# dalek-cryptography/curve25519-dalek

Measured on NVIDIA H100. Metric: Pippenger MSM points/sec, higher is better.
Workload: dtype exact integers: f64 limbs (radix 2^51, FP64 pipe) in the bucket kernel, u32 limbs (radix 2^25.5) elsewhere

## Files before the change

### curve25519_dalek_b200/csrc/fe64.cuh

```cuda
#pragma once
#include <stdint.h>

#include "fe.cuh"

struct fe64 { double v[5]; };

#define FE64_E52 0x4330000000000000LL
#define FE64_TWO52 4503599627370496.0
#define FE64_TWO51 2251799813685248.0

#if defined(__CUDA_ARCH__)
#define FE64_DEV 1
#else
#define FE64_DEV 0
#include <assert.h>
#include <math.h>
#include <string.h>
#endif

FE_HD void fe64_0(fe64 &h) { for (int i = 0; i < 5; i++) h.v[i] = 0.0; }
FE_HD void fe64_1(fe64 &h) { h.v[0] = 1.0; for (int i = 1; i < 5; i++) h.v[i] = 0.0; }

FE_HD void fe64_add(fe64 &h, const fe64 &f, const fe64 &g)
{
#pragma unroll
    for (int i = 0; i < 5; i++) h.v[i] = f.v[i] + g.v[i];
}
FE_HD void fe64_sub(fe64 &h, const fe64 &f, const fe64 &g)
{
#pragma unroll
    for (int i = 0; i < 5; i++) h.v[i] = f.v[i] - g.v[i];
}

FE_HD void fe64_cmov(fe64 &h, const fe64 &g, uint32_t c)
{
#if FE64_DEV
#pragma unroll
    for (int i = 0; i < 5; i++) {
        long long a = __double_as_longlong(h.v[i]), b = __double_as_longlong(g.v[i]);
        long long m = 0LL - (long long)c;
        h.v[i] = __longlong_as_double(a ^ (m & (a ^ b)));
    }
#else
    if (c) h = g;
#endif
}

#if !FE64_DEV
static inline void fe64_assert_scale(const fe64 &f, double s)
{
    for (int i = 0; i < 5; i++) {
        assert(f.v[i] == floor(f.v[i]));
        assert(fabs(f.v[i]) <= s * 1125899906842624.0 + 32768.0 * s);
    }
}
#define FE64_ASSERT_SCALE(f, s) fe64_assert_scale((f), (s))
#else
#define FE64_ASSERT_SCALE(f, s) ((void)0)
#endif

FE_HD void fe64_finish(fe64 &h, long long V[9])
{
    long long R[5];
#pragma unroll
    for (int k = 0; k < 4; k++) R[k] = V[k] + 19 * V[k + 5];
    R[4] = V[4];
    const long long HALF = 1LL << 50;
    long long c;
    c = (R[0] + HALF) >> 51; R[0] -= c * (1LL << 51); R[1] += c;
    c = (R[1] + HALF) >> 51; R[1] -= c * (1LL << 51); R[2] += c;
    c = (R[2] + HALF) >> 51; R[2] -= c * (1LL << 51); R[3] += c;
    c = (R[3] + HALF) >> 51; R[3] -= c * (1LL << 51); R[4] += c;
    c = (R[4] + HALF) >> 51; R[4] -= c * (1LL << 51); R[0] += 19 * c;
    c = (R[0] + HALF) >> 51; R[0] -= c * (1LL << 51); R[1] += c;
#pragma unroll
    for (int k = 0; k < 5; k++) {
#if FE64_DEV
        h.v[k] = __longlong_as_double((R[k] + (1LL << 51)) | FE64_E52) - (FE64_TWO52 + FE64_TWO51);
#else
        h.v[k] = (double)R[k];
#endif
    }
}

FE_HD void fe64_mul(fe64 &h, const fe64 &a, const fe64 &b)
{
    long long V[9];
#if FE64_DEV
    const double M1 = 6755399441055744.0;
    const double K = 6755399441055744.0 * 4503599627370496.0 + 4503599627370496.0;
    double bs[5];
#pragma unroll
    for (int j = 0; j < 5; j++) bs[j] = b.v[j] * (1.0 / 4503599627370496.0);
    long long H[10], L[9];
#pragma unroll
    for (int k = 0; k < 10; k++) H[k] = 0;
#pragma unroll
    for (int k = 0; k < 9; k++) L[k] = 0;
#pragma unroll
    for (int i = 0; i < 5; i++)
#pragma unroll
        for (int j = 0; j < 5; j++) {
            double t = __fma_rz(a.v[i], bs[j], M1);
            double u = __fma_rn(t, -4503599627370496.0, K);
            double lo = __fma_rn(a.v[i], b.v[j], u);
            H[i + j + 1] += __double_as_longlong(t);
            L[i + j] += __double_as_longlong(lo);
        }
    const long long EH = FE64_E52 + (1LL << 51);
#pragma unroll
    for (int k = 0; k < 9; k++) {
        const int nl = k < 5 ? k + 1 : 9 - k;
        const int nh = k == 0 ? 0 : (k <= 5 ? k : 10 - k);
        V[k] = (L[k] - nl * FE64_E52) + 2 * (H[k] - nh * EH);
    }
    V[4] += 38 * (H[9] - EH);
#else
    for (int k = 0; k < 9; k++) V[k] = 0;
    long long V9 = 0;
    for (int i = 0; i < 5; i++)
        for (int j = 0; j < 5; j++) {
            __int128 p = (__int128)(long long)a.v[i] * (__int128)(long long)b.v[j];
            __int128 lim = (__int128)1 << 103;
            assert(p < lim && p > -lim);
            long long f = (long long)(p >> 52);
            long long lo = (long long)(p - ((__int128)f << 52));
            V[i + j] += lo;
            if (i + j + 1 < 9) V[i + j + 1] += 2 * f; else V9 += 2 * f;
        }
    V[4] += 19 * V9;
#endif
    fe64_finish(h, V);
}

FE_HD void fe64_sq(fe64 &h, const fe64 &a)
{
    long long V[9];
#if FE64_DEV
    const double M1 = 6755399441055744.0;
    const double K = 6755399441055744.0 * 4503599627370496.0 + 4503599627370496.0;
    double as[5], a2[5];
#pragma unroll
    for (int j = 0; j < 5; j++) { as[j] = a.v[j] * (1.0 / 4503599627370496.0); a2[j] = a.v[j] + a.v[j]; }
    long long H[10], L[9];
#pragma unroll
    for (int k = 0; k < 10; k++) H[k] = 0;
#pragma unroll
    for (int k = 0; k < 9; k++) L[k] = 0;
#pragma unroll
    for (int i = 0; i < 5; i++)
#pragma unroll
        for (int j = i; j < 5; j++) {
            const double x = i < j ? a2[i] : a.v[i];
            double t = __fma_rz(x, as[j], M1);
            double u = __fma_rn(t, -4503599627370496.0, K);
            double lo = __fma_rn(x, a.v[j], u);
            H[i + j + 1] += __double_as_longlong(t);
            L[i + j] += __double_as_longlong(lo);
        }
    const long long EH = FE64_E52 + (1LL << 51);
#pragma unroll
    for (int k = 0; k < 9; k++) {
        const int nl = k < 5 ? k / 2 + 1 : (8 - k) / 2 + 1;
        const int km = k - 1;
        const int nh = k == 0 ? 0 : (km < 5 ? km / 2 + 1 : (8 - km) / 2 + 1);
        V[k] = (L[k] - nl * FE64_E52) + 2 * (H[k] - nh * EH);
    }
    V[4] += 38 * (H[9] - EH);
#else
    for (int k = 0; k < 9; k++) V[k] = 0;
    long long V9 = 0;
    for (int i = 0; i < 5; i++)
        for (int j = i; j < 5; j++) {
            __int128 p = (__int128)(long long)a.v[i] * (__int128)(long long)a.v[j] * (i < j ? 2 : 1);
            __int128 lim = (__int128)1 << 103;
            assert(p < lim && p > -lim);
            long long f = (long long)(p >> 52);
            long long lo = (long long)(p - ((__int128)f << 52));
            V[i + j] += lo;
            if (i + j + 1 < 9) V[i + j + 1] += 2 * f; else V9 += 2 * f;
        }
    V[4] += 19 * V9;
#endif
    fe64_finish(h, V);
}

FE_HD void fe64_sqn(fe64 &h, const fe64 &f, int n)
{
    fe64_sq(h, f);
#if FE64_DEV
#pragma unroll 1
#endif
    for (int i = 1; i < n; i++) fe64_sq(h, h);
}

FE_HD void fe64_carry(fe64 &h, const fe64 &f)
{
#if FE64_DEV
    const double C = 6755399441055744.0;
    double q[5], r[5];
#pragma unroll
    for (int k = 0; k < 5; k++) {
        q[k] = __fma_rn(f.v[k], 1.0 / 2251799813685248.0, C) - C;
        r[k] = __fma_rn(q[k], -2251799813685248.0, f.v[k]);
    }
    h.v[0] = __fma_rn(q[4], 19.0, r[0]);
#pragma unroll
    for (int k = 1; k < 5; k++) h.v[k] = r[k] + q[k - 1];
#else
    double q[5], r[5];
    for (int k = 0; k < 5; k++) { q[k] = nearbyint(f.v[k] / 2251799813685248.0); r[k] = f.v[k] - q[k] * 2251799813685248.0; }
    h.v[0] = r[0] + 19.0 * q[4];
    for (int k = 1; k < 5; k++) h.v[k] = r[k] + q[k - 1];
#endif
}

FE_HD void fe64_frombytes_words(fe64 &h, const uint32_t w[8])
{
    uint64_t l[5];
    l[0] = (uint64_t)w[0] | ((uint64_t)(w[1] & 0x7ffffu) << 32);
    l[1] = (uint64_t)(w[1] >> 19) | ((uint64_t)w[2] << 13) | ((uint64_t)(w[3] & 0x3fu) << 45);
    l[2] = (uint64_t)(w[3] >> 6) | ((uint64_t)(w[4] & 0x1ffffffu) << 26);
    l[3] = (uint64_t)(w[4] >> 25) | ((uint64_t)w[5] << 7) | ((uint64_t)(w[6] & 0xfffu) << 39);
    l[4] = (uint64_t)(w[6] >> 12) | ((uint64_t)(w[7] & 0x7fffffffu) << 20);
#pragma unroll
    for (int k = 0; k < 5; k++) {
#if FE64_DEV
        h.v[k] = __longlong_as_double((long long)l[k] | FE64_E52) - FE64_TWO52;
#else
        h.v[k] = (double)l[k];
#endif
    }
}

FE_HD void fe64_to_fe(fe &o, const fe64 &f)
{
    uint64_t l[5];
#pragma unroll
    for (int k = 0; k < 5; k++) {
        long long r = (long long)f.v[k];
        l[k] = (uint64_t)(r + (k == 0 ? (1LL << 54) - 152 : (1LL << 54) - 8));
    }
    uint64_t c[10];
#pragma unroll
    for (int i = 0; i < 5; i++) { c[2 * i] = l[i] & FE_M26; c[2 * i + 1] = l[i] >> 26; }
    fe_carry64(o, c);
}

FE_HD void fe64_from_fe(fe64 &h, const fe &f)
{
    uint32_t w[8];
    fe_tobytes_words(w, f);
    fe64 t; fe64_frombytes_words(t, w);
    fe64_carry(h, t);
}

FE_HD void fe64_pow22501(fe64 &t19, fe64 &t3, const fe64 &z)
{
    fe64 t0, t1, t2, t5, t6, t7, t9, t13, t15;
    fe64_sq(t0, z);
    fe64_sqn(t1, t0, 2);
    fe64_mul(t2, z, t1);
    fe64_mul(t3, t0, t2);
    fe64_sq(t1, t3);
    fe64_mul(t5, t2, t1);
    fe64_sqn(t6, t5, 5);    fe64_mul(t7, t6, t5);
    fe64_sqn(t6, t7, 10);   fe64_mul(t9, t6, t7);
    fe64_sqn(t6, t9, 20);   fe64_mul(t6, t6, t9);
    fe64_sqn(t6, t6, 10);   fe64_mul(t13, t6, t7);
    fe64_sqn(t6, t13, 50);  fe64_mul(t15, t6, t13);
    fe64_sqn(t6, t15, 100); fe64_mul(t6, t6, t15);
    fe64_sqn(t6, t6, 50);   fe64_mul(t19, t6, t13);
}

FE_HD void fe_pow_p58_f64(fe &h, const fe &f)
{
    fe64 z, t19, t3;
    fe64_from_fe(z, f);
    fe64_pow22501(t19, t3, z);
    fe64_sqn(t19, t19, 2);
    fe64_mul(t19, z, t19);
    fe64_to_fe(h, t19);
}

FE_HD void fe_invert_f64(fe &h, const fe &f)
{
    fe64 z, t19, t3;
    fe64_from_fe(z, f);
    fe64_pow22501(t19, t3, z);
    fe64_sqn(t19, t19, 5);
    fe64_mul(t19, t19, t3);
    fe64_to_fe(h, t19);
}
```

### curve25519_dalek_b200/csrc/ge64.cuh

```cuda
#pragma once
#include "fe64.cuh"
#include "ge.cuh"

struct ge64_p3 { fe64 X, Y, Z, T; };
struct ge64_niels { fe64 ypx, ymx, xy2d; };
struct ge64_pniels { fe64 YpX, YmX, Z, T2d; };

FE_HD void ge64_identity(ge64_p3 &p) { fe64_0(p.X); fe64_1(p.Y); fe64_1(p.Z); fe64_0(p.T); }

FE_HD void ge64_niels_unpack(ge64_niels &n, const ge_niels_packed &o)
{
    fe64_frombytes_words(n.ypx, o.w); fe64_frombytes_words(n.ymx, o.w + 8); fe64_frombytes_words(n.xy2d, o.w + 16);
}
FE_HD void ge64_pniels_unpack(ge64_pniels &n, const ge_pniels_packed &o)
{
    fe64_frombytes_words(n.YpX, o.w); fe64_frombytes_words(n.YmX, o.w + 8);
    fe64_frombytes_words(n.Z, o.w + 16); fe64_frombytes_words(n.T2d, o.w + 24);
}

FE_HD void ge64_add_tail(ge64_p3 &r, const fe64 &a, const fe64 &b, const fe64 &c, const fe64 &D, uint32_t neg)
{
    fe64 E, H, DpC, DmC, F, G;
    fe64_sub(E, b, a);
    fe64_add(H, b, a);
    fe64_add(DpC, D, c);
    fe64_sub(DmC, D, c);
    fe64_carry(DmC, DmC);
    F = DmC; fe64_cmov(F, DpC, neg);
    G = DpC; fe64_cmov(G, DmC, neg);
    fe64_mul(r.X, F, E);
    fe64_mul(r.Y, G, H);
    fe64_mul(r.Z, DmC, DpC);
    fe64_mul(r.T, E, H);
}

FE_HD void ge64_madd(ge64_p3 &r, const ge64_p3 &p, const ge64_niels &q, uint32_t neg)
{
    FE64_ASSERT_SCALE(p.X, 1); FE64_ASSERT_SCALE(p.Y, 1); FE64_ASSERT_SCALE(p.Z, 1); FE64_ASSERT_SCALE(p.T, 1);
    fe64 A, B, a, b, c, D;
    fe64 qp = q.ypx, qm = q.ymx;
    { fe64 t = qp; fe64_cmov(qp, qm, neg); fe64_cmov(qm, t, neg); }
    fe64_sub(A, p.Y, p.X);
    fe64_add(B, p.Y, p.X);
    fe64_mul(a, A, qm);
    fe64_mul(b, B, qp);
    fe64_mul(c, p.T, q.xy2d);
    fe64_add(D, p.Z, p.Z);
    ge64_add_tail(r, a, b, c, D, neg);
}

FE_HD void ge64_padd(ge64_p3 &r, const ge64_p3 &p, const ge64_pniels &q, uint32_t neg)
{
    FE64_ASSERT_SCALE(p.X, 1); FE64_ASSERT_SCALE(p.Y, 1); FE64_ASSERT_SCALE(p.Z, 1); FE64_ASSERT_SCALE(p.T, 1);
    fe64 A, B, a, b, c, ZZ, D;
    fe64 qp = q.YpX, qm = q.YmX;
    { fe64 t = qp; fe64_cmov(qp, qm, neg); fe64_cmov(qm, t, neg); }
    fe64_sub(A, p.Y, p.X);
    fe64_add(B, p.Y, p.X);
    fe64_mul(a, A, qm);
    fe64_mul(b, B, qp);
    fe64_mul(c, p.T, q.T2d);
    fe64_mul(ZZ, p.Z, q.Z);
    fe64_add(D, ZZ, ZZ);
    ge64_add_tail(r, a, b, c, D, neg);
}

template <bool T_OUT = true>
FE_HD void ge64_dbl(ge64_p3 &r, const ge64_p3 &p)
{
    FE64_ASSERT_SCALE(p.X, 1); FE64_ASSERT_SCALE(p.Y, 1); FE64_ASSERT_SCALE(p.Z, 1);
    fe64 XX, YY, ZZ, XpY, XpY2, Yp, Ym, E, F;
    fe64_sq(XX, p.X);
    fe64_sq(YY, p.Y);
    fe64_sq(ZZ, p.Z);
    fe64_add(XpY, p.X, p.Y); fe64_carry(XpY, XpY);
    fe64_sq(XpY2, XpY);
    fe64_add(Yp, YY, XX);
    fe64_sub(Ym, YY, XX);
    fe64_sub(E, XpY2, Yp);
    fe64_add(F, ZZ, ZZ); fe64_sub(F, F, Ym);
    fe64_carry(F, F);
    fe64_mul(r.X, E, F);
    fe64_mul(r.Y, Yp, Ym);
    fe64_mul(r.Z, Ym, F);
    if (T_OUT) fe64_mul(r.T, E, Yp);
}

FE_HD void ge64_add_p3(ge64_p3 &r, const ge64_p3 &p, const ge64_p3 &q, const fe64 &d2)
{
    ge64_pniels pn;
    fe64_add(pn.YpX, q.Y, q.X);
    fe64_sub(pn.YmX, q.Y, q.X);
    pn.Z = q.Z;
    fe64_mul(pn.T2d, q.T, d2);
    ge64_padd(r, p, pn, 0u);
}

FE_HD void ge64_from_p3(ge64_p3 &o, const ge_p3 &p)
{
    fe64_from_fe(o.X, p.X); fe64_from_fe(o.Y, p.Y); fe64_from_fe(o.Z, p.Z); fe64_from_fe(o.T, p.T);
}

FE_HD void ge64_to_p3(ge_p3 &o, const ge64_p3 &p)
{
    fe64_to_fe(o.X, p.X); fe64_to_fe(o.Y, p.Y); fe64_to_fe(o.Z, p.Z); fe64_to_fe(o.T, p.T);
}
```

### curve25519_dalek_b200/csrc/msm.cu

```cuda
#include <algorithm>
#include <cstdio>
#include <utility>
#include <vector>

#include "../../include/dalek_b200.h"
#include "engine.h"
#include "ge64.cuh"
#include "warp4.cuh"
#include "warp4_f64.cuh"

static inline unsigned cdiv(size_t a, unsigned b) { return (unsigned)((a + b - 1) / b); }

int ws_reserve(dalek_b200_ctx *ctx, DevBuf &b, size_t bytes)
{
    if (bytes <= b.cap) return 0;
    if (b.p) { cudaFree(b.p); b.p = nullptr; b.cap = 0; }
    size_t want = bytes + bytes / 8 + 256;
    cudaError_t e = cudaMalloc(&b.p, want);
    if (e != cudaSuccess) {
        ctx->last_error = std::string("cudaMalloc: ") + cudaGetErrorString(e);
        (void)cudaGetLastError();
        return DALEK_E_NOMEM;
    }
    b.cap = want;
// ... 496 lines not shown
{
    extern __shared__ uint32_t sm[];
    __shared__ uint32_t s_bin, s_slice;
    uint2 *recs = reinterpret_cast<uint2 *>(sm);
    uint32_t *out = sm + 2 * SORT_FINE_CAP, *h = out + SORT_FINE_CAP, *scr = h + (1u << F);
    const uint32_t nf = 1u << F, nbins = nwin * nc;
    uint32_t bin, slice = 0;
    if (blockIdx.x < nbins) {
        bin = nbins - 1 - blockIdx.x;
    } else {
        if (threadIdx.x == 0) {
            uint32_t t = blockIdx.x - nbins, w = 0;
            while (w < nwin && t >= xtot[w]) t -= xtot[w++];
            s_bin = nbins;
            if (w < nwin) {
                const uint32_t *x = xpre + (size_t)w * nc;
                uint32_t lo = 0, hi = nc - 1;
                while (lo < hi) { const uint32_t mid = (lo + hi + 1) / 2; if (x[mid] <= t) lo = mid; else hi = mid - 1; }
                s_bin = w * nc + lo;
                s_slice = t - x[lo] + 1;
            }
        }
        __syncthreads();
        bin = s_bin; slice = s_slice;
        if (bin >= nbins) return;
    }
    const uint32_t wb = bin / nc, cb = bin % nc;
    const uint32_t cnt = ccount[bin], base = ccursor[bin] - cnt;
    const size_t seg = flat ? (size_t)0 : (size_t)wb * n;
    const size_t b0 = (size_t)wb * nbuckets + ((size_t)cb << F);
    const uint2 *src = records + seg + base;
    uint32_t *dst = sorted + seg + base;
    constexpr uint32_t U = 4;
    if (cnt <= SORT_FINE_CAP) {
        for (uint32_t f = threadIdx.x; f < nf; f += SORT_THREADS) h[f] = 0;
        __syncthreads();
        for (uint32_t k0 = 0; k0 < cnt; k0 += U * SORT_THREADS) {
            uint2 r[U];
#pragma unroll
            for (uint32_t u = 0; u < U; u++) {
                const uint32_t k = k0 + u * SORT_THREADS + threadIdx.x;
                r[u] = k < cnt ? src[k] : make_uint2(0, 0);
            }
#pragma unroll
            for (uint32_t u = 0; u < U; u++) {
                const uint32_t k = k0 + u * SORT_THREADS + threadIdx.x;
                if (k < cnt) { recs[k] = r[u]; atomicAdd(&h[r[u].y], 1u); }
            }
        }
        __syncthreads();
        for (uint32_t f = threadIdx.x; f < nf; f += SORT_THREADS) counts[b0 + f] = h[f];
        block_excl_scan(h, nf, scr);
        for (uint32_t f = threadIdx.x; f < nf; f += SORT_THREADS) offsets[b0 + f] = base + h[f];
        __syncthreads();
        for (uint32_t k = threadIdx.x; k < cnt; k += SORT_THREADS) { const uint2 r = recs[k]; out[atomicAdd(&h[r.y], 1u)] = r.x; }
        __syncthreads();
        for (uint32_t k = threadIdx.x; k < cnt; k += SORT_THREADS) dst[k] = out[k];
        return;
    }
    for (uint32_t f = threadIdx.x; f < nf; f += SORT_THREADS) { h[f] = counts[b0 + f]; out[f] = 0; }
    block_excl_scan(h, nf, scr);
    if (slice == 0)
        for (uint32_t f = threadIdx.x; f < nf; f += SORT_THREADS) offsets[b0 + f] = base + h[f];
    const uint32_t lo = slice * SORT_FINE_CAP, m = min(SORT_FINE_CAP, cnt - lo);
    for (uint32_t k0 = 0; k0 < m; k0 += U * SORT_THREADS) {
        uint2 r[U];
#pragma unroll
        for (uint32_t u = 0; u < U; u++) {
            const uint32_t k = k0 + u * SORT_THREADS + threadIdx.x;
            r[u] = k < m ? src[lo + k] : make_uint2(0, 0);
        }
#pragma unroll
        for (uint32_t u = 0; u < U; u++) {
            const uint32_t k = k0 + u * SORT_THREADS + threadIdx.x;
            if (k < m) recs[k] = r[u];
            warp_claim(out, r[u].y, k < m);
        }
    }
    __syncthreads();
    for (uint32_t f = threadIdx.x; f < nf; f += SORT_THREADS)
        if (out[f]) out[f] = h[f] + atomicAdd(&fill[b0 + f], out[f]);
    __syncthreads();
    for (uint32_t k0 = 0; k0 < m; k0 += SORT_THREADS) {
        const uint32_t k = k0 + threadIdx.x;
        const uint2 r = k < m ? recs[k] : make_uint2(0, 0);
        const uint32_t pos = warp_claim(out, r.y, k < m);
        if (k < m) dst[pos] = r.x;
    }
}

#define SCAN_PART 4096u
__global__ void __launch_bounds__(1024) k_scan_partial(const uint32_t *__restrict__ in, uint32_t nbuckets, uint32_t parts,
                                                       uint32_t *__restrict__ part_sums)
{
    __shared__ uint32_t sh[32];
    uint32_t w = blockIdx.x / parts, part = blockIdx.x % parts;
    const uint32_t *src = in + (size_t)w * nbuckets;
    uint32_t base = part * SCAN_PART + threadIdx.x * 4, sum = 0;
#pragma unroll
    for (int k = 0; k < 4; k++) if (base + k < nbuckets) sum += src[base + k];
    for (int d = 16; d > 0; d >>= 1) sum += __shfl_down_sync(0xffffffffu, sum, d);
    if ((threadIdx.x & 31) == 0) sh[threadIdx.x >> 5] = sum;
    __syncthreads();
    if (threadIdx.x < 32) {
        uint32_t v = sh[threadIdx.x];
        for (int d = 16; d > 0; d >>= 1) v += __shfl_down_sync(0xffffffffu, v, d);
        if (threadIdx.x == 0) part_sums[blockIdx.x] = v;
    }
}
__global__ void k_scan_bases(uint32_t *__restrict__ part_sums, uint32_t parts)
{
    if (threadIdx.x) return;
    uint32_t *p = part_sums + (size_t)blockIdx.x * parts, run = 0;
    for (uint32_t k = 0; k < parts; k++) { uint32_t v = p[k]; p[k] = run; run += v; }
}
__global__ void __launch_bounds__(1024) k_scan_apply(const uint32_t *__restrict__ in, const uint32_t *__restrict__ part_base,
                                                     uint32_t nbuckets, uint32_t parts, uint32_t *__restrict__ out)
{
    __shared__ uint32_t sh[32];
    uint32_t w = blockIdx.x / parts, part = blockIdx.x % parts;
    const uint32_t *src = in + (size_t)w * nbuckets;
    uint32_t *dst = out + (size_t)w * nbuckets;
    uint32_t base = part * SCAN_PART + threadIdx.x * 4;
    uint32_t v[4], sum = 0;
#pragma unroll
    for (int k = 0; k < 4; k++) { v[k] = base + k < nbuckets ? src[base + k] : 0; sum += v[k]; }
    uint32_t incl = sum;
    for (int d = 1; d < 32; d <<= 1) { uint32_t t = __shfl_up_sync(0xffffffffu, incl, d); if ((threadIdx.x & 31) >= d) incl += t; }
    if ((threadIdx.x & 31) == 31) sh[threadIdx.x >> 5] = incl;
    __syncthreads();
    if (threadIdx.x < 32) {
        uint32_t x = sh[threadIdx.x], inc2 = x;
        for (int d = 1; d < 32; d <<= 1) { uint32_t t = __shfl_up_sync(0xffffffffu, inc2, d); if (threadIdx.x >= d) inc2 += t; }
        sh[threadIdx.x] = inc2 - x;
    }
    __syncthreads();
    uint32_t run = part_base[blockIdx.x] + sh[threadIdx.x >> 5] + incl - sum;
#pragma unroll
    for (int k = 0; k < 4; k++) { if (base + k < nbuckets) dst[base + k] = run; run += v[k]; }
}

#define TASK_LEN_MIN 64u
static uint32_t msm_task_len(size_t n, int nwin, uint32_t nb)
{
    const size_t total_buckets = (size_t)nwin * nb;
    const size_t want = total_buckets >= ((size_t)1 << 18) ? 2 * (n / nb) : (n * (size_t)nwin) >> 18;
    uint32_t len = TASK_LEN_MIN;
    while (len < want && len < (1u << 22)) len <<= 1;
    return len;
}
#ifndef ACC_MIN_BLOCKS
#define ACC_MIN_BLOCKS 4
#endif

__global__ void k_task_count(const uint32_t *__restrict__ counts, uint32_t total_buckets, uint32_t task_len,
                             uint32_t *__restrict__ ntasks, uint32_t *__restrict__ heavy)
{
    uint32_t t = blockIdx.x * blockDim.x + threadIdx.x;
    if (t >= total_buckets) return;
    uint32_t c = counts[t];
    uint32_t k = c <= task_len ? 1u : (c + task_len - 1) / task_len;
    ntasks[t] = k;
    if (k > 1) heavy[1 + atomicAdd(&heavy[0], 1u)] = t;
}

__global__ void k_task_bases(const uint32_t *__restrict__ ntasks, const uint32_t *__restrict__ task_off, uint32_t nbuckets,
                             int nwin, uint32_t *__restrict__ win_base )
{
    if (blockIdx.x || threadIdx.x) return;
    uint32_t run = 0;
    for (int w = 0; w < nwin; w++) {
        win_base[w] = run;
        size_t last = (size_t)w * nbuckets + nbuckets - 1;
        run += task_off[last] + ntasks[last];
    }
    win_base[nwin] = run;
}

__global__ void k_task_fill(const uint32_t *__restrict__ ntasks, const uint32_t *__restrict__ task_off,
                            const uint32_t *__restrict__ win_base, uint32_t nbuckets, uint32_t total_buckets,
                            uint2 *__restrict__ tasks)
{
    uint32_t t = blockIdx.x * blockDim.x + threadIdx.x;
    if (t >= total_buckets) return;
    uint32_t w = t / nbuckets;
    uint32_t base = win_base[w] + task_off[t], k = ntasks[t];
    for (uint32_t j = 0; j < k; j++) tasks[base + j] = make_uint2(t, j);
}

#define TASK_BINS 256u
__device__ __forceinline__ uint32_t task_key(uint32_t len, uint32_t task_len)
{
    return (uint32_t)(((uint64_t)len * (TASK_BINS - 1) + task_len - 1) / task_len);
}
__device__ __forceinline__ uint32_t task_length(const uint2 tk, const uint32_t *__restrict__ counts, uint32_t task_len)
{
    return min(task_len, counts[tk.x] - tk.y * task_len);
}

__global__ void __launch_bounds__(256)
k_task_hist(const uint2 *__restrict__ tasks, const uint32_t *__restrict__ counts, const uint32_t *__restrict__ total_ptr,
            uint32_t task_len, uint32_t *__restrict__ hist)
{
    __shared__ uint32_t sh[TASK_BINS];
    sh[threadIdx.x] = 0;
    __syncthreads();
    const uint32_t p = blockIdx.x * blockDim.x + threadIdx.x;
    if (p < *total_ptr) atomicAdd(&sh[task_key(task_length(tasks[p], counts, task_len), task_len)], 1u);
    __syncthreads();
    if (sh[threadIdx.x]) atomicAdd(&hist[threadIdx.x], sh[threadIdx.x]);
}

__global__ void __launch_bounds__(256) k_task_scan(const uint32_t *__restrict__ hist, uint32_t *__restrict__ start)
{
    __shared__ uint32_t sh[TASK_BINS];
    const uint32_t k = TASK_BINS - 1 - threadIdx.x;
    sh[threadIdx.x] = hist[k];
    __syncthreads();
    for (uint32_t d = 1; d < TASK_BINS; d <<= 1) {
        uint32_t v = threadIdx.x >= d ? sh[threadIdx.x - d] : 0;
        __syncthreads();
        sh[threadIdx.x] += v;
        __syncthreads();
    }
    start[k] = sh[threadIdx.x] - hist[k];
}

__global__ void __launch_bounds__(256)
k_task_scatter(const uint2 *__restrict__ tasks, const uint32_t *__restrict__ counts, const uint32_t *__restrict__ total_ptr,
               uint32_t task_len, const uint32_t *__restrict__ start, uint32_t *__restrict__ cursor, uint32_t *__restrict__ order)
{
    __shared__ uint32_t cnt[TASK_BINS], base[TASK_BINS];
    cnt[threadIdx.x] = 0;
    __syncthreads();
    const uint32_t p = blockIdx.x * blockDim.x + threadIdx.x;
    const bool live = p < *total_ptr;
    uint32_t key = 0, rank = 0;
    if (live) { key = task_key(task_length(tasks[p], counts, task_len), task_len); rank = atomicAdd(&cnt[key], 1u); }
    __syncthreads();
    if (cnt[threadIdx.x]) base[threadIdx.x] = start[threadIdx.x] + atomicAdd(&cursor[threadIdx.x], cnt[threadIdx.x]);
    __syncthreads();
    if (live) order[base[key] + rank] = p;
}

__device__ __forceinline__ void load_p3(ge_p3 &p, const ge_p3_raw *src)
{
    const uint4 *s = reinterpret_cast<const uint4 *>(src);
    ge_p3_raw r;
#pragma unroll
    for (int q = 0; q < 10; q++) { uint4 v = s[q]; r.w[4 * q] = v.x; r.w[4 * q + 1] = v.y; r.w[4 * q + 2] = v.z; r.w[4 * q + 3] = v.w; }
    ge_p3_load_raw(p, r);
}

template <int F64, int TMA>
__global__ void __launch_bounds__(128, ACC_MIN_BLOCKS)
k_bucket_accumulate(const ge_niels_packed *__restrict__ points, const uint32_t *__restrict__ sorted,
                    const uint32_t *__restrict__ counts, const uint32_t *__restrict__ offsets,
                    const uint32_t *__restrict__ ntasks, const uint2 *__restrict__ tasks, const uint32_t *__restrict__ order,
                    const uint32_t *__restrict__ win_base, int w0, int w1, size_t n, uint32_t nbuckets, uint32_t task_len,
                    ge_p3_raw *__restrict__ buckets, ge_p3_raw *__restrict__ task_sums, int first)
{
    constexpr int NQ = sizeof(ge_niels_packed) / 16;
    constexpr int TSTRIDE = NQ * 16 + 16;
    __shared__ uint4 s_pts[(F64 && !TMA) ? 2 : 1][(F64 && !TMA) ? NQ : 1][(F64 && !TMA) ? 128 : 1];
    __shared__ __align__(16) unsigned char s_bulk[(F64 && TMA) ? 2 : 1][(F64 && TMA) ? 128 : 1][(F64 && TMA) ? TSTRIDE : 16];
    __shared__ __align__(8) unsigned long long s_bar[(F64 && TMA) ? 2 : 1][(F64 && TMA) ? 128 : 1];
    const uint32_t total_tasks = win_base[w1];
    const uint32_t slot = blockIdx.x * 128u + threadIdx.x;
    if (slot >= total_tasks) return;
    const uint32_t p = order[slot];
    const uint2 tk = tasks[p];
    const uint32_t t = tk.x, w = t / nbuckets;
    const uint32_t cnt = counts[t], start = tk.y * task_len;
    const uint32_t len = min(task_len, cnt - start);
    const bool split = ntasks[t] != 1;
    if (!first && len == 0) return;
    const bool fold_old = !first && !split;
    const uint32_t *idx = sorted + (size_t)w * n + offsets[t] + start;
    ge_p3 acc;
    if (F64) {
        ge64_p3 acc64;
        if (fold_old) {
            ge_p3 old; load_p3(old, buckets + t);
            fe64_from_fe(acc64.X, old.X); fe64_from_fe(acc64.Y, old.Y); fe64_from_fe(acc64.Z, old.Z); fe64_from_fe(acc64.T, old.T);
        } else {
            ge64_identity(acc64);
        }
        uint32_t e_next = len ? idx[0] : 0;
        if (TMA) {
            const uint32_t bar0 = (uint32_t)__cvta_generic_to_shared(&s_bar[0][threadIdx.x]);
            const uint32_t bar1 = (uint32_t)__cvta_generic_to_shared(&s_bar[1][threadIdx.x]);
            asm volatile("mbarrier.init.shared::cta.b64 [%0], 1;" ::"r"(bar0) : "memory");
            asm volatile("mbarrier.init.shared::cta.b64 [%0], 1;" ::"r"(bar1) : "memory");
            asm volatile("fence.mbarrier_init.release.cluster;" ::: "memory");
            asm volatile("fence.proxy.async.shared::cta;" ::: "memory");
        }
        auto prefetch = [&](uint32_t e, int buf) {
            const uint32_t pi = e & 0x7fffffffu;
            const char *src = reinterpret_cast<const char *>(points) + (size_t)pi * (NQ * 16);
            if (TMA) {
                const uint32_t bar = (uint32_t)__cvta_generic_to_shared(&s_bar[buf][threadIdx.x]);
                const uint32_t dst = (uint32_t)__cvta_generic_to_shared(&s_bulk[buf][threadIdx.x][0]);
                asm volatile("mbarrier.arrive.expect_tx.shared::cta.b64 _, [%0], %1;" ::"r"(bar), "r"(NQ * 16) : "memory");
                asm volatile("cp.async.bulk.shared::cluster.global.mbarrier::complete_tx::bytes [%0], [%1], %2, [%3];"
                             ::"r"(dst), "l"(src), "r"(NQ * 16), "r"(bar) : "memory");
            } else {
#pragma unroll
                for (int q = 0; q < NQ; q++) {
                    uint32_t dst = (uint32_t)__cvta_generic_to_shared(&s_pts[buf][q][threadIdx.x]);
                    asm volatile("cp.async.cg.shared.global [%0], [%1], 16;" ::"r"(dst), "l"(src + 16 * q) : "memory");
                }
            }
        };
        if (len) prefetch(e_next, 0);
        if (!TMA) asm volatile("cp.async.commit_group;" ::: "memory");
        for (uint32_t k = 0; k < len; k++) {
            const uint32_t e = e_next, neg = e >> 31;
            const int buf = k & 1;
            if (k + 1 < len) { e_next = idx[k + 1]; prefetch(e_next, buf ^ 1); }
            uint32_t words[NQ * 4];
            if (TMA) {
                const uint32_t bar = (uint32_t)__cvta_generic_to_shared(&s_bar[buf][threadIdx.x]);
                const uint32_t parity = (k >> 1) & 1u;
                uint32_t done;
                do {
                    asm volatile("{ .reg .pred p; mbarrier.try_wait.parity.shared::cta.b64 p, [%1], %2; selp.u32 %0, 1, 0, p; }"
                                 : "=r"(done) : "r"(bar), "r"(parity) : "memory");
                } while (!done);
                const uint4 *sp = reinterpret_cast<const uint4 *>(&s_bulk[buf][threadIdx.x][0]);
#pragma unroll
                for (int q = 0; q < NQ; q++) { uint4 v = sp[q]; words[4 * q] = v.x; words[4 * q + 1] = v.y; words[4 * q + 2] = v.z; words[4 * q + 3] = v.w; }
            } else {
                asm volatile("cp.async.commit_group;" ::: "memory");
                asm volatile("cp.async.wait_group 1;" ::: "memory");
#pragma unroll
                for (int q = 0; q < NQ; q++) { uint4 v = s_pts[buf][q][threadIdx.x]; words[4 * q] = v.x; words[4 * q + 1] = v.y; words[4 * q + 2] = v.z; words[4 * q + 3] = v.w; }
            }
            ge_niels_packed pk;
#pragma unroll
            for (int q = 0; q < 24; q++) pk.w[q] = words[q];
            ge64_niels nl; ge64_niels_unpack(nl, pk);
            ge64_madd(acc64, acc64, nl, neg);
        }
        ge64_to_p3(acc, acc64);
    } else {
    if (fold_old) load_p3(acc, buckets + t); else ge_p3_identity(acc);
    for (uint32_t k = 0; k < len; k++) {
        uint32_t e = idx[k];
        uint32_t neg = e >> 31, pi = e & 0x7fffffffu;
        const uint4 *src = reinterpret_cast<const uint4 *>(reinterpret_cast<const ge_niels_packed *>(points) + pi);
        ge_niels_packed pk;
#pragma unroll
        for (int q = 0; q < 6; q++) { uint4 v = __ldg(src + q); pk.w[4 * q] = v.x; pk.w[4 * q + 1] = v.y; pk.w[4 * q + 2] = v.z; pk.w[4 * q + 3] = v.w; }
        ge_niels nl; ge_niels_unpack(nl, pk);
        ge_madd(acc, acc, nl, neg);
    }
    }
    ge_p3_raw r; ge_p3_store_raw(r, acc);
    uint4 *o = reinterpret_cast<uint4 *>(!split ? buckets + t : task_sums + p);
#pragma unroll
    for (int q = 0; q < 10; q++) o[q] = make_uint4(r.w[4 * q], r.w[4 * q + 1], r.w[4 * q + 2], r.w[4 * q + 3]);
}


__global__ void __launch_bounds__(128)
k_heavy_fixup(const uint32_t *__restrict__ heavy, const uint32_t *__restrict__ ntasks, const uint32_t *__restrict__ task_off,
              const uint32_t *__restrict__ win_base, uint32_t nbuckets, uint32_t w0, uint32_t w1,
              const ge_p3_raw *__restrict__ task_sums, ge_p3_raw *__restrict__ buckets, int first)
{
    const uint32_t lane = threadIdx.x & 31, role = lane & 3, grp = lane >> 2;
    const uint32_t nwarps = (gridDim.x * blockDim.x) >> 5;
    const uint32_t nheavy = heavy[0];
    for (uint32_t h = (blockIdx.x * blockDim.x + threadIdx.x) >> 5; h < nheavy; h += nwarps) {
        uint32_t tb = heavy[1 + h];
        if (tb / nbuckets < w0 || tb / nbuckets >= w1) continue;
        uint32_t kk = ntasks[tb];
        uint32_t base = win_base[tb / nbuckets] + task_off[tb];
        w4_point acc, x;
        if (first || grp != 0) w4_identity(acc); else w4_load(acc, buckets + tb);
        for (uint32_t j0 = 0; j0 < kk; j0 += 8) {
            uint32_t j = j0 + grp;
            if (j < kk) w4_load(x, task_sums + base + j); else w4_identity(x);
            w4_add(acc, x, role);
        }
        for (int d = 16; d >= 4; d >>= 1) { w4_shfl_down(x, acc, d); w4_add(acc, x, role); }
        if (grp == 0) w4_store(buckets + tb, acc, role);
    }
}

__device__ __forceinline__ void load_p3_f64(ge64_p3 &o, const ge_p3_raw *src)
{
    ge_p3 q; load_p3(q, src);
    fe64_from_fe_limbs(o.X, q.X); fe64_from_fe_limbs(o.Y, q.Y); fe64_from_fe_limbs(o.Z, q.Z); fe64_from_fe_limbs(o.T, q.T);
}

__global__ void __launch_bounds__(32)
k_chunk_reduce_f64(const ge_p3_raw *__restrict__ S_in, uint32_t n_in, uint32_t m, uint32_t n_out, uint32_t nwin,
                   ge_p3_raw *__restrict__ S_out, ge_p3_raw *__restrict__ W_out)
{
    const uint32_t t = blockIdx.x * blockDim.x + threadIdx.x;
    if (t >= n_out * nwin) return;
    const uint32_t w = t / n_out, q = t % n_out;
    const ge_p3_raw *S = S_in + (size_t)w * n_in + (size_t)q * m;
    fe64 d2; fe64_const_2d(d2);
    ge64_p3 run, acc, x;
    load_p3_f64(run, S + (m - 1));
    acc = run;
    ge_p3 nxt;
    if (m > 1) load_p3(nxt, S + (m - 2));
#pragma unroll 1
    for (uint32_t r = m - 1; r-- > 0;) {
        fe64_from_fe_limbs(x.X, nxt.X); fe64_from_fe_limbs(x.Y, nxt.Y); fe64_from_fe_limbs(x.Z, nxt.Z); fe64_from_fe_limbs(x.T, nxt.T);
        if (r > 0) load_p3(nxt, S + (r - 1));
        ge64_add_p3(run, run, x, d2);
        ge64_add_p3(acc, acc, run, d2);
    }
    ge_p3 o; ge_p3_raw raw;
    ge64_to_p3(o, run); ge_p3_store_raw(raw, o);
    uint4 *d = reinterpret_cast<uint4 *>(S_out + t);
#pragma unroll
    for (int k = 0; k < 10; k++) d[k] = make_uint4(raw.w[4 * k], raw.w[4 * k + 1], raw.w[4 * k + 2], raw.w[4 * k + 3]);
    ge64_to_p3(o, acc); ge_p3_store_raw(raw, o);
    d = reinterpret_cast<uint4 *>(W_out + t);
#pragma unroll
    for (int k = 0; k < 10; k++) d[k] = make_uint4(raw.w[4 * k], raw.w[4 * k + 1], raw.w[4 * k + 2], raw.w[4 * k + 3]);
}

__global__ void __launch_bounds__(128)
k_chunk_reduce(const ge_p3_raw *__restrict__ S_in, uint32_t n_in, uint32_t m, uint32_t one_based, uint32_t n_out,
               uint32_t nwin, ge_p3_raw *__restrict__ S_out, ge_p3_raw *__restrict__ W_out)
{
    const uint32_t t = (blockIdx.x * blockDim.x + threadIdx.x) >> 5;
    if (t >= n_out * nwin) return;
    const w20_role rl = w20_roles();
    const double d2 = w20_const_2d(rl);
    const uint32_t w = t / n_out, q = t % n_out;
    const ge_p3_raw *S = S_in + (size_t)w * n_in + (size_t)q * m;
    double run = w20_load(S + (m - 1), rl), acc = run;
#pragma unroll 1
    for (uint32_t r = m - 1; r-- > 1;) {
        w20_add(run, w20_load(S + r, rl), d2, rl);
        w20_add(acc, run, d2, rl);
    }
    if (m > 1) {
        w20_add(run, w20_load(S, rl), d2, rl);
        if (one_based) w20_add(acc, run, d2, rl);
    } else if (!one_based) {
        acc = w20_identity(rl);
    }
    w20_store(S_out + t, run);
    w20_store(W_out + t, acc);
}

#define SUM_PIECE 256u
__global__ void __launch_bounds__(128)
k_plain_sum(const ge_p3_raw *__restrict__ pool, const uint2 *__restrict__ desc, ge_p3_raw *__restrict__ out)
{
    __shared__ ge_p3_raw sh[32];
    const uint32_t role = threadIdx.x & 3, grp = threadIdx.x >> 2;
    const uint2 d = desc[blockIdx.x];
    const ge_p3_raw *a = pool + d.x;
    const uint32_t len = d.y;
    w4_point acc, x;
    w4_identity(acc);
    for (uint32_t i0 = 0; i0 < len; i0 += 32) {
        uint32_t i = i0 + grp;
        if (i < len) w4_load(x, a + i); else w4_identity(x);
        w4_add(acc, x, role);
    }
    w4_store(&sh[grp], acc, role);
    __syncthreads();
    for (uint32_t d = 16; d > 0; d >>= 1) {
        if (threadIdx.x < 32 * ((d + 7) / 8)) {
            uint32_t g2 = grp < d ? grp + d : grp;
            w4_load(acc, &sh[grp]); w4_load(x, &sh[g2]);
            w4_add(acc, x, role);
        }
        __syncthreads();
        if (grp < d) w4_store(&sh[grp], acc, role);
        __syncthreads();
    }
    if (grp == 0) { w4_load(acc, &sh[0]); w4_store(out + blockIdx.x, acc, role); }
}

struct LevelInfo { int nlevels; int log2m[16]; };
__global__ void __launch_bounds__(128)
k_finish_windows(const ge_p3_raw *__restrict__ S_top, const ge_p3_raw *__restrict__ A, LevelInfo li, uint32_t nwin,
                 ge_p3_raw *__restrict__ out)
{
    const uint32_t w = (blockIdx.x * blockDim.x + threadIdx.x) >> 5;
    if (w >= nwin) return;
    const w20_role rl = w20_roles();
    double t;
    if (li.nlevels > 0) {
        const double d2 = w20_const_2d(rl);
// ... 217 lines not shown
```

Baseline: 373.0 million.

## Generalize bucket gather prefetch ring and streamline f64 madd arithmetic

Replaces the fixed double-buffered point prefetch with a configurable-depth ring (ACC_PF, default 1), which keeps the same depth but changes index bookkeeping to a register ring with lookahead index loads. The mixed addition now uses a sign-multiplier formulation, folding the negation into fma operations instead of cmov swaps. Its first three multiplies use a parallel, non-serial carry in the finish step. Limb unpacking now uses funnel shifts and hi/lo double construction instead of 64-bit shifts. It also adds a gather probe mode for experiments, off by default. Risks include looser limb bounds from the parallel carry and extra registers from the index ring.

```diff
diff --git a/curve25519_dalek_b200/csrc/fe64.cuh b/curve25519_dalek_b200/csrc/fe64.cuh
--- a/curve25519_dalek_b200/csrc/fe64.cuh
+++ b/curve25519_dalek_b200/csrc/fe64.cuh
@@ -59,6 +59,7 @@
 #define FE64_ASSERT_SCALE(f, s) ((void)0)
 #endif
 
+template <bool PAR = false>
 FE_HD void fe64_finish(fe64 &h, long long V[9])
 {
     long long R[5];
@@ -66,13 +67,22 @@
     for (int k = 0; k < 4; k++) R[k] = V[k] + 19 * V[k + 5];
     R[4] = V[4];
     const long long HALF = 1LL << 50;
-    long long c;
-    c = (R[0] + HALF) >> 51; R[0] -= c * (1LL << 51); R[1] += c;
-    c = (R[1] + HALF) >> 51; R[1] -= c * (1LL << 51); R[2] += c;
-    c = (R[2] + HALF) >> 51; R[2] -= c * (1LL << 51); R[3] += c;
-    c = (R[3] + HALF) >> 51; R[3] -= c * (1LL << 51); R[4] += c;
-    c = (R[4] + HALF) >> 51; R[4] -= c * (1LL << 51); R[0] += 19 * c;
-    c = (R[0] + HALF) >> 51; R[0] -= c * (1LL << 51); R[1] += c;
+    if (PAR) {
+        long long c[5];
+#pragma unroll
+        for (int k = 0; k < 5; k++) { c[k] = (R[k] + HALF) >> 51; R[k] -= c[k] * (1LL << 51); }
+        R[0] += 19 * c[4];
+#pragma unroll
+        for (int k = 1; k < 5; k++) R[k] += c[k - 1];
+    } else {
+        long long c;
+        c = (R[0] + HALF) >> 51; R[0] -= c * (1LL << 51); R[1] += c;
+        c = (R[1] + HALF) >> 51; R[1] -= c * (1LL << 51); R[2] += c;
+        c = (R[2] + HALF) >> 51; R[2] -= c * (1LL << 51); R[3] += c;
+        c = (R[3] + HALF) >> 51; R[3] -= c * (1LL << 51); R[4] += c;
+        c = (R[4] + HALF) >> 51; R[4] -= c * (1LL << 51); R[0] += 19 * c;
+        c = (R[0] + HALF) >> 51; R[0] -= c * (1LL << 51); R[1] += c;
+    }
 #pragma unroll
     for (int k = 0; k < 5; k++) {
 #if FE64_DEV
@@ -83,6 +93,7 @@
     }
 }
 
+template <bool PAR = false>
 FE_HD void fe64_mul(fe64 &h, const fe64 &a, const fe64 &b)
 {
     long long V[9];
@@ -130,7 +141,7 @@
         }
     V[4] += 19 * V9;
 #endif
-    fe64_finish(h, V);
+    fe64_finish<PAR>(h, V);
 }
 
 FE_HD void fe64_sq(fe64 &h, const fe64 &a)
@@ -217,20 +228,22 @@
 
 FE_HD void fe64_frombytes_words(fe64 &h, const uint32_t w[8])
 {
+#if FE64_DEV
+    const uint32_t HI = (uint32_t)(FE64_E52 >> 32), M19 = 0x7ffffu;
+    const uint32_t lo[5] = {w[0], __funnelshift_r(w[1], w[2], 19), __funnelshift_r(w[3], w[4], 6),
+                            __funnelshift_r(w[4], w[5], 25), __funnelshift_r(w[6], w[7], 12)};
+    const uint32_t hi[5] = {w[1], __funnelshift_r(w[2], w[3], 19), w[4] >> 6, __funnelshift_r(w[5], w[6], 25), w[7] >> 12};
+#pragma unroll
+    for (int k = 0; k < 5; k++) h.v[k] = __hiloint2double((int)((hi[k] & M19) | HI), (int)lo[k]) - FE64_TWO52;
+#else
     uint64_t l[5];
     l[0] = (uint64_t)w[0] | ((uint64_t)(w[1] & 0x7ffffu) << 32);
     l[1] = (uint64_t)(w[1] >> 19) | ((uint64_t)w[2] << 13) | ((uint64_t)(w[3] & 0x3fu) << 45);
     l[2] = (uint64_t)(w[3] >> 6) | ((uint64_t)(w[4] & 0x1ffffffu) << 26);
     l[3] = (uint64_t)(w[4] >> 25) | ((uint64_t)w[5] << 7) | ((uint64_t)(w[6] & 0xfffu) << 39);
     l[4] = (uint64_t)(w[6] >> 12) | ((uint64_t)(w[7] & 0x7fffffffu) << 20);
-#pragma unroll
-    for (int k = 0; k < 5; k++) {
-#if FE64_DEV
-        h.v[k] = __longlong_as_double((long long)l[k] | FE64_E52) - FE64_TWO52;
-#else
-        h.v[k] = (double)l[k];
-#endif
-    }
+    for (int k = 0; k < 5; k++) h.v[k] = (double)l[k];
+#endif
 }
 
 FE_HD void fe64_to_fe(fe &o, const fe64 &f)
diff --git a/curve25519_dalek_b200/csrc/ge64.cuh b/curve25519_dalek_b200/csrc/ge64.cuh
--- a/curve25519_dalek_b200/csrc/ge64.cuh
+++ b/curve25519_dalek_b200/csrc/ge64.cuh
@@ -47,6 +47,35 @@
     fe64_mul(c, p.T, q.xy2d);
     fe64_add(D, p.Z, p.Z);
     ge64_add_tail(r, a, b, c, D, neg);
+}
+
+FE_HD void ge64_madd_signed(ge64_p3 &r, const ge64_p3 &p, const ge64_niels &q, uint32_t neg)
+{
+    FE64_ASSERT_SCALE(p.X, 1); FE64_ASSERT_SCALE(p.Y, 1); FE64_ASSERT_SCALE(p.Z, 1); FE64_ASSERT_SCALE(p.T, 1);
+#if FE64_DEV
+    const double s = __longlong_as_double(0x3ff0000000000000LL | ((long long)neg << 63));
+#else
+    const double s = neg ? -1.0 : 1.0;
+#endif
+    fe64 A, B, a, b, c, E, H, F, G;
+#pragma unroll
+    for (int i = 0; i < 5; i++) { A.v[i] = fma(-s, p.X.v[i], p.Y.v[i]); B.v[i] = fma(s, p.X.v[i], p.Y.v[i]); }
+    fe64_mul<true>(a, A, q.ymx);
+    fe64_mul<true>(b, B, q.ypx);
+    fe64_mul<true>(c, p.T, q.xy2d);
+#pragma unroll
+    for (int i = 0; i < 5; i++) {
+        const double D = p.Z.v[i] + p.Z.v[i];
+        E.v[i] = (b.v[i] - a.v[i]) * s;
+        H.v[i] = b.v[i] + a.v[i];
+        F.v[i] = fma(-s, c.v[i], D);
+        G.v[i] = fma(s, c.v[i], D);
+    }
+    fe64_carry(F, F);
+    fe64_mul(r.X, E, F);
+    fe64_mul(r.Y, G, H);
+    fe64_mul(r.Z, F, G);
+    fe64_mul(r.T, E, H);
 }
 
 FE_HD void ge64_padd(ge64_p3 &r, const ge64_p3 &p, const ge64_pniels &q, uint32_t neg)
diff --git a/curve25519_dalek_b200/csrc/msm.cu b/curve25519_dalek_b200/csrc/msm.cu
--- a/curve25519_dalek_b200/csrc/msm.cu
+++ b/curve25519_dalek_b200/csrc/msm.cu
@@ -672,6 +672,12 @@
 #ifndef ACC_MIN_BLOCKS
 #define ACC_MIN_BLOCKS 4
 #endif
+#ifndef ACC_PF
+#define ACC_PF 1
+#endif
+#ifndef ACC_GATHER_PROBE
+#define ACC_GATHER_PROBE 0
+#endif
 
 __global__ void k_task_count(const uint32_t *__restrict__ counts, uint32_t total_buckets, uint32_t task_len,
                              uint32_t *__restrict__ ntasks, uint32_t *__restrict__ heavy)
@@ -782,9 +788,10 @@
 {
     constexpr int NQ = sizeof(ge_niels_packed) / 16;
     constexpr int TSTRIDE = NQ * 16 + 16;
-    __shared__ uint4 s_pts[(F64 && !TMA) ? 2 : 1][(F64 && !TMA) ? NQ : 1][(F64 && !TMA) ? 128 : 1];
-    __shared__ __align__(16) unsigned char s_bulk[(F64 && TMA) ? 2 : 1][(F64 && TMA) ? 128 : 1][(F64 && TMA) ? TSTRIDE : 16];
-    __shared__ __align__(8) unsigned long long s_bar[(F64 && TMA) ? 2 : 1][(F64 && TMA) ? 128 : 1];
+    constexpr int PF = ACC_PF, NS = ACC_PF + 1;
+    __shared__ uint4 s_pts[(F64 && !TMA) ? NS : 1][(F64 && !TMA) ? NQ : 1][(F64 && !TMA) ? 128 : 1];
+    __shared__ __align__(16) unsigned char s_bulk[(F64 && TMA) ? NS : 1][(F64 && TMA) ? 128 : 1][(F64 && TMA) ? TSTRIDE : 16];
+    __shared__ __align__(8) unsigned long long s_bar[(F64 && TMA) ? NS : 1][(F64 && TMA) ? 128 : 1];
     const uint32_t total_tasks = win_base[w1];
     const uint32_t slot = blockIdx.x * 128u + threadIdx.x;
     if (slot >= total_tasks) return;
@@ -806,16 +813,19 @@
         } else {
             ge64_identity(acc64);
         }
-        uint32_t e_next = len ? idx[0] : 0;
+        uint32_t ring[PF + 2];
+#pragma unroll
+        for (int j = 0; j < PF + 2; j++) ring[j] = (uint32_t)j < len ? idx[j] : 0u;
         if (TMA) {
-            const uint32_t bar0 = (uint32_t)__cvta_generic_to_shared(&s_bar[0][threadIdx.x]);
-            const uint32_t bar1 = (uint32_t)__cvta_generic_to_shared(&s_bar[1][threadIdx.x]);
-            asm volatile("mbarrier.init.shared::cta.b64 [%0], 1;" ::"r"(bar0) : "memory");
-            asm volatile("mbarrier.init.shared::cta.b64 [%0], 1;" ::"r"(bar1) : "memory");
+#pragma unroll
+            for (int j = 0; j < NS; j++) {
+                const uint32_t bar = (uint32_t)__cvta_generic_to_shared(&s_bar[j][threadIdx.x]);
+                asm volatile("mbarrier.init.shared::cta.b64 [%0], 1;" ::"r"(bar) : "memory");
+            }
             asm volatile("fence.mbarrier_init.release.cluster;" ::: "memory");
             asm volatile("fence.proxy.async.shared::cta;" ::: "memory");
         }
-        auto prefetch = [&](uint32_t e, int buf) {
+        auto prefetch = [&](uint32_t e, uint32_t buf) {
             const uint32_t pi = e & 0x7fffffffu;
             const char *src = reinterpret_cast<const char *>(points) + (size_t)pi * (NQ * 16);
             if (TMA) {
@@ -832,27 +842,59 @@
                 }
             }
         };
-        if (len) prefetch(e_next, 0);
-        if (!TMA) asm volatile("cp.async.commit_group;" ::: "memory");
+#pragma unroll
+        for (int j = 0; j < PF; j++) {
+            if ((uint32_t)j < len) prefetch(ring[j], j);
+            if (!TMA) asm volatile("cp.async.commit_group;" ::: "memory");
+        }
+#if ACC_GATHER_PROBE
+        if (len) {
+            asm volatile("cp.async.wait_all;" ::: "memory");
+            if (TMA) {
+                uint32_t done;
+                do {
+                    asm volatile("{ .reg .pred p; mbarrier.try_wait.parity.shared::cta.b64 p, [%1], 0; selp.u32 %0, 1, 0, p; }"
+                                 : "=r"(done) : "r"((uint32_t)__cvta_generic_to_shared(&s_bar[0][threadIdx.x])) : "memory");
+                } while (!done);
+            }
+        }
+#endif
+        uint32_t cur = 0, nxt = PF;
         for (uint32_t k = 0; k < len; k++) {
-            const uint32_t e = e_next, neg = e >> 31;
-            const int buf = k & 1;
-            if (k + 1 < len) { e_next = idx[k + 1]; prefetch(e_next, buf ^ 1); }
+#if ACC_GATHER_PROBE
+            const uint32_t neg = k & 1u;
+#if ACC_GATHER_PROBE == 2
+            const ge64_niels self = {acc64.Y, acc64.X, acc64.T};
+            ge64_madd_signed(acc64, acc64, self, neg);
+            continue;
+#endif
+            const uint32_t buf = 0;
+#else
+            const uint32_t neg = ring[0] >> 31, buf = cur;
+            if (k + PF < len) prefetch(ring[PF], nxt);
+#pragma unroll
+            for (int j = 0; j < PF + 1; j++) ring[j] = ring[j + 1];
+            ring[PF + 1] = k + PF + 2 < len ? idx[k + PF + 2] : 0u;
+            nxt = cur; cur = cur + 1 == NS ? 0 : cur + 1;
+#endif
             uint32_t words[NQ * 4];
             if (TMA) {
-                const uint32_t bar = (uint32_t)__cvta_generic_to_shared(&s_bar[buf][threadIdx.x]);
-                const uint32_t parity = (k >> 1) & 1u;
-                uint32_t done;
-                do {
-                    asm volatile("{ .reg .pred p; mbarrier.try_wait.parity.shared::cta.b64 p, [%1], %2; selp.u32 %0, 1, 0, p; }"
-                                 : "=r"(done) : "r"(bar), "r"(parity) : "memory");
-                } while (!done);
+                if (!ACC_GATHER_PROBE) {
+                    const uint32_t bar = (uint32_t)__cvta_generic_to_shared(&s_bar[buf][threadIdx.x]);
+                    uint32_t done;
+                    do {
+                        asm volatile("{ .reg .pred p; mbarrier.try_wait.parity.shared::cta.b64 p, [%1], %2; selp.u32 %0, 1, 0, p; }"
+                                     : "=r"(done) : "r"(bar), "r"((k / NS) & 1u) : "memory");
+                    } while (!done);
+                }
                 const uint4 *sp = reinterpret_cast<const uint4 *>(&s_bulk[buf][threadIdx.x][0]);
 #pragma unroll
                 for (int q = 0; q < NQ; q++) { uint4 v = sp[q]; words[4 * q] = v.x; words[4 * q + 1] = v.y; words[4 * q + 2] = v.z; words[4 * q + 3] = v.w; }
             } else {
-                asm volatile("cp.async.commit_group;" ::: "memory");
-                asm volatile("cp.async.wait_group 1;" ::: "memory");
+                if (!ACC_GATHER_PROBE) {
+                    asm volatile("cp.async.commit_group;" ::: "memory");
+                    asm volatile("cp.async.wait_group %0;" ::"n"(PF) : "memory");
+                }
 #pragma unroll
                 for (int q = 0; q < NQ; q++) { uint4 v = s_pts[buf][q][threadIdx.x]; words[4 * q] = v.x; words[4 * q + 1] = v.y; words[4 * q + 2] = v.z; words[4 * q + 3] = v.w; }
             }
@@ -860,7 +902,7 @@
 #pragma unroll
             for (int q = 0; q < 24; q++) pk.w[q] = words[q];
             ge64_niels nl; ge64_niels_unpack(nl, pk);
-            ge64_madd(acc64, acc64, nl, neg);
+            ge64_madd_signed(acc64, acc64, nl, neg);
         }
         ge64_to_p3(acc, acc64);
     } else {
```

Result: faster. 388.0 million, median of 6 (+4.0%).
